# LessUp/gpu-spmv

Hardware: AMD Instinct MI355X
Metric: spmv_effective_bandwidth (higher is better)
Workload: dtype f32; 1 GPU; csr_uniform_10000000x10000000_16_per_row_pagerank_step; rows=10000000, cols=10000000, nnz=160000000, avg_nnz_per_row=16, plan_bytes=1798181216, parallelism=row-shard x1, exchange=none

## Files before the change

### gpu-spmv_amd/csrc/capi.cpp

```cpp
#include "internal.h"
#include "generators.h"
#include "pagerank_engine.h"
#include "tiled.h"
#include "spmv/bandwidth.h"
#include "spmv/bicgstab.h"
#include "spmv/gmres.h"
#include "spmv/eigs.h"
#include "spmv/cg.h"
#include "spmv/pagerank.h"
#include "spmv/sptrsv.h"
#include "spmv/ic0.h"
#include "spmv/ilu0.h"
#include "spmv/spgemm.h"
#include "spmv/amg.h"
#include "spmv/reorder.h"
#include "spmv_c.h"

#include <cstddef>
#include <cstring>
#include <vector>
#include <new>

using namespace spmv;

// ... 856 lines not shown
    sh.local_rows = A->num_rows;
    sh.map = map;
    sh.n_global = n_global;
    sh.nnz = A->nnz;
    sh.d_row_ptrs = A->d_row_ptrs;
    sh.d_cols = A->d_col_indices;
    sh.d_vals = A->d_values;
    sh.d_dangling = d_dangling_mask;
    const int partial_pairs = detail::pr_shard_prepare(&sh, detail::tiled_plan_for(A, nullptr));
    if (hipMalloc(reinterpret_cast<void**>(&sh.d_state), sizeof(detail::PrState)) != hipSuccess ||
        hipMalloc(reinterpret_cast<void**>(&sh.d_block_partials),
                  2 * sizeof(double) * static_cast<size_t>(partial_pairs)) != hipSuccess) {
        spmv_c_pr_shard_destroy(h);
        return nullptr;
    }
    return h;
}

void spmv_c_pr_shard_destroy(spmv_c_pr_shard* h) {
    if (!h) return;
    if (h->shard.commit_pending) {
        (void)detail::pr_flush(h->shard, h->shard.pending_stream);
        (void)hipGetLastError();
    }
    if (h->shard.d_state) (void)hipFree(h->shard.d_state);
    if (h->shard.d_block_partials) (void)hipFree(h->shard.d_block_partials);
    delete h;
}

int spmv_c_pr_reset(spmv_c_pr_shard* h, float dangling_sum, void* hip_stream) {
    if (!h) return kInvalidArgument;
    detail::PrState fresh{};
    fresh.dangling_sum = dangling_sum;
    h->shard.expanded_strips = 0;
    h->shard.expanded_long = false;
    detail::pr_drop_pending(h->shard);
    return hipMemcpyAsync(h->shard.d_state, &fresh, sizeof(fresh), hipMemcpyHostToDevice,
                          as_stream(hip_stream)) == hipSuccess
         ? 0 : static_cast<int>(SpMVError::CUDA_MEMCPY);
}

int spmv_c_pr_step(spmv_c_pr_shard* h, const float* d_r_old, float* d_r_new, float damping,
                   void* hip_stream) {
    if (!h || !d_r_old || !d_r_new) return kInvalidArgument;
    return launch_code(detail::pr_step(h->shard, d_r_old, d_r_new, damping, detail::PushTargets{},
                                       as_stream(hip_stream)));
}

int spmv_c_pr_step_commit(spmv_c_pr_shard* h, const float* d_r_old, float* d_r_new, float damping,
                          float tolerance, void* hip_stream) {
    if (!h || !d_r_old || !d_r_new) return kInvalidArgument;
// ... 117 lines not shown
```

### gpu-spmv_amd/csrc/pagerank.hip

```cpp
#include "internal.h"
#include "device_common.h"
#include "pagerank_engine.h"
#include "pr_commit_device.h"
#include "tiled.h"
#include "spmv/pagerank.h"

#include <hip/hip_runtime.h>

#include <algorithm>
#include <chrono>
#include <cmath>
#include <cstdio>
#include <cstdlib>
#include <cstring>
#include <mutex>
#include <vector>

namespace spmv {
namespace detail {

namespace {

using namespace dev;

// ... 122 lines not shown
__global__ __launch_bounds__(kBlock)
void pr_mask_kernel(const float* __restrict__ col_sums, int n, unsigned char* __restrict__ mask,
                    unsigned long long* __restrict__ count) {
    unsigned long long local = 0;
    for (long long c = static_cast<long long>(blockIdx.x) * kBlock + threadIdx.x; c < n;
         c += static_cast<long long>(gridDim.x) * kBlock) {
        const bool d = col_sums[c] == 0.0f;
        mask[c] = d;
        local += d;
    }
    for (int off = 32; off > 0; off >>= 1) local += __shfl_xor(local, off, 64);
    if ((threadIdx.x & 63) == 0 && local) atomicAdd(count, local);
}

__global__ __launch_bounds__(kBlock)
void pr_vector_sum_kernel(const float* __restrict__ v, size_t n, double* __restrict__ block_out) {
    double acc = 0.0, unused = 0.0;
    for (size_t i = static_cast<size_t>(blockIdx.x) * kBlock + threadIdx.x; i < n;
         i += static_cast<size_t>(gridDim.x) * kBlock) {
        acc += static_cast<double>(v[i]);
    }
    block_sum2<kBlock>(acc, unused);
    if (threadIdx.x == 0) block_out[blockIdx.x] = acc;
}

__global__ __launch_bounds__(kBlock)
void pr_scale_kernel(float* __restrict__ v, size_t n, const double* __restrict__ block_sums, int blocks) {
    __shared__ float s_total;
    if (threadIdx.x == 0) {
        double total = 0.0;
// ... 90 lines not shown
    } else if (const hipError_t e = pr_flush(sh, s); e != hipSuccess) {
        return e;
    }
    if (sh.local_rows <= 0) return hipSuccess;
    if (sh.tiled) {
        const int done = std::min(sh.expanded_strips, sh.tiled->num_strips);
        const bool long_done = sh.expanded_long;
        sh.expanded_strips = 0;
        sh.expanded_long = false;
        std::unique_lock<std::mutex> pair(sh.tiled->launch_lock, std::defer_lock);
        if (done == 0 && !long_done) pair.lock();
        if (done < sh.tiled->num_strips || !long_done) {
            const hipError_t e = tiled_pagerank_expand(*sh.tiled, done, sh.tiled->num_strips, !long_done, r_old, sh.d_state, rider, s);
            if (e != hipSuccess) return e;
        }
        return tiled_pagerank_finish(*sh.tiled, sh.map, sh.n_global, r_old, r_new, sh.d_dangling,
                                     damping, sh.d_state, sh.d_block_partials, push, s);
    }
    switch (sh.lanes) {
        case 1:  return launch_step<1>(sh, r_old, r_new, damping, push, s);
        case 2:  return launch_step<2>(sh, r_old, r_new, damping, push, s);
        case 4:  return launch_step<4>(sh, r_old, r_new, damping, push, s);
        case 8:  return launch_step<8>(sh, r_old, r_new, damping, push, s);
        case 16: return launch_step<16>(sh, r_old, r_new, damping, push, s);
        case 32: return launch_step<32>(sh, r_old, r_new, damping, push, s);
        default: return launch_step<64>(sh, r_old, r_new, damping, push, s);
    }
}

hipError_t pr_expand(const PrShard& sh, const float* r_old, long long cols_ready, hipStream_t s) {
    if (const hipError_t e = pr_flush(sh, s); e != hipSuccess) return e;
// ... 40 lines not shown
    pr_reduce_commit_kernel<<<1, kBlock, 0, s>>>(sh.d_block_partials, sh.local_rows > 0 ? sh.grid : 0, tolerance,
                                                 sh.d_state);
    return hipGetLastError();
}

hipError_t pr_commit(const PrShard& sh, const double* d_sums, float tolerance, hipStream_t s) {
    if (const hipError_t e = pr_flush(sh, s); e != hipSuccess) return e;
    pr_commit_kernel<<<1, 1, 0, s>>>(d_sums, tolerance, sh.d_state);
    return hipGetLastError();
}

hipError_t pr_commit_gathered(const PrShard& sh, const float* d_gathered, int world, long long stride,
                              long long shard_len, float tolerance, hipStream_t s) {
    if (const hipError_t e = pr_flush(sh, s); e != hipSuccess) return e;
    pr_commit_gathered_kernel<<<1, 1, 0, s>>>(d_gathered, world, stride, shard_len, tolerance, sh.d_state);
    return hipGetLastError();
}

hipError_t pr_fill(float* d_r, size_t n, float value, hipStream_t s) {
    if (n == 0) return hipSuccess;
    pr_fill_kernel<<<grid_for(static_cast<long long>(n), kBlock * 4), kBlock, 0, s>>>(d_r, n, value);
    return hipGetLastError();
}

hipError_t pr_column_sums(long long nnz, const int* d_cols, const float* d_vals, int n_cols,
                          float* d_col_sums, hipStream_t s) {
    if (nnz == 0) return hipSuccess;
    pr_colsum_kernel<<<grid_for(nnz, kBlock * 4), kBlock, 0, s>>>(nnz, d_cols, d_vals, n_cols, d_col_sums);
    return hipGetLastError();
}
// ... 463 lines not shown
```

### gpu-spmv_amd/csrc/pagerank_engine.h

```cpp
#ifndef SPMV_AMD_PAGERANK_ENGINE_H
#define SPMV_AMD_PAGERANK_ENGINE_H

#include "internal.h"

namespace spmv {
namespace detail {

struct PrState {
    float dangling_sum;
    float final_residual;
    int   iterations;
    int   converged;
    int   done;
    int   reserved;
};

constexpr int kMaxPushPeers = 15;
struct PushTargets {
    float* ptr[kMaxPushPeers];
    int count = 0;
};

struct RowMap {
    int base = 0;
    int piece = 0x7fffffff;
    int block = 0;
    __host__ __device__ long long at(long long row) const {
        return piece == 0x7fffffff ? base + row : base + (row / piece) * block + row % piece;
    }
};

struct PrShard {
    int local_rows = 0;
    RowMap map;
    int n_global = 0;
    long long nnz = 0;
    const int* d_row_ptrs = nullptr;
    const int* d_cols = nullptr;
    const float* d_vals = nullptr;
    const unsigned char* d_dangling = nullptr;
    PrState* d_state = nullptr;
    double* d_block_partials = nullptr;
    int lanes = 4;
    int grid = 1;
    PlanRef tiled;
    mutable int expanded_strips = 0;
    mutable bool expanded_long = false;
    mutable bool commit_pending = false;
    mutable float pending_tolerance = 0.0f;
    mutable hipStream_t pending_stream = nullptr;
};

struct CommitRider {
    const double* partials = nullptr;
    int num_blocks = 0;
// ... 3 lines not shown

int pr_max_blocks();
int pr_shard_prepare(PrShard* shard, PlanRef tiled);
hipError_t pr_step(const PrShard& shard, const float* d_r_old, float* d_r_new, float damping,
                   const PushTargets& push, hipStream_t s);
hipError_t pr_expand(const PrShard& shard, const float* d_r_old, long long cols_ready, hipStream_t s);
hipError_t pr_reduce(const PrShard& shard, double* d_sums , hipStream_t s);
hipError_t pr_commit(const PrShard& shard, const double* d_sums, float tolerance, hipStream_t s);
hipError_t pr_reduce_commit(const PrShard& shard, float tolerance, hipStream_t s);
hipError_t pr_step_commit(const PrShard& shard, const float* d_r_old, float* d_r_new, float damping,
                          float tolerance, hipStream_t s);
hipError_t pr_flush(const PrShard& shard, hipStream_t s);
inline void pr_drop_pending(const PrShard& shard) { shard.commit_pending = false; }
hipError_t pr_commit_gathered(const PrShard& shard, const float* d_gathered, int world, long long stride,
                              long long shard_len, float tolerance, hipStream_t s);
hipError_t pr_fill(float* d_r, size_t n, float value, hipStream_t s);
hipError_t pr_column_sums(long long nnz, const int* d_cols, const float* d_vals, int n_cols,
                          float* d_col_sums, hipStream_t s);
hipError_t pr_mask_from_column_sums(const float* d_col_sums, int n, unsigned char* d_mask,
                                    unsigned long long* d_count, hipStream_t s);

}
}

#endif
```

### gpu-spmv_amd/csrc/tiled.h

```cpp
#ifndef SPMV_AMD_TILED_H
#define SPMV_AMD_TILED_H

#include "internal.h"

#include <cstdint>
#include <mutex>
#include <vector>

namespace spmv {
namespace detail {

struct PrState;
struct CommitRider;
struct PushTargets;
struct RowMap;
struct PassDesc;

struct TiledPlan {
    int num_rows = 0, num_cols = 0;
    long long nnz = 0;
    long long entries = 0;
    int strip_cols = 0;
    int tile_rows = 0;
    int num_strips = 0, num_tiles = 0;

    DevBuf<float>    a_val;
    DevBuf<float>    col_weight;
    DevBuf<uint16_t> a_lcol;
    DevBuf<uint8_t>  a_drow;
    DevBuf<float>    prod;
    DevBuf<int>      cells_t;
    DevBuf<int>      pass_first;
    DevBuf<PassDesc> pass_desc;
    long long num_passes = 0;

    DevBuf<int> items;
    int  num_items = 0;
    std::vector<int> strip_first_item;
    DevBuf<int>   long_rows;
    int    num_long = 0;
    int    long_row = 1024;
    DevBuf<int>   long_chunks;
    int    num_long_chunks = 0;
    DevBuf<int>   long_first;
    DevBuf<float> long_sums;
    DevBuf<int>   tile_long;
    const int*   csr_row_ptrs = nullptr;
    const int*   csr_cols = nullptr;
// ... 21 lines not shown
bool tiled_eligible(const CSRMatrix* A);
bool tiled_eligible(const ELLMatrix* A);

hipError_t tiled_build(const CSRMatrix* A, TiledPlan** out, hipStream_t s);
hipError_t tiled_build(const ELLMatrix* A, TiledPlan** out, hipStream_t s);
void tiled_free(TiledPlan* plan);

hipError_t tiled_checksum(const TiledPlan& plan, unsigned long long out[4], hipStream_t s);

hipError_t tiled_spmv(const TiledPlan& plan, const float* d_x, float* d_y, hipStream_t s);

hipError_t tiled_pagerank_expand(const TiledPlan& plan, int strip_begin, int strip_end, bool with_long,
                                 const float* d_r_old, const PrState* d_state, const CommitRider& commit, hipStream_t s);
hipError_t tiled_pagerank_finish(const TiledPlan& plan, const RowMap& map, int n_global,
                                 const float* d_r_old, float* d_r_new,
                                 const unsigned char* d_dangling, float damping,
                                 const PrState* d_state, double* d_block_partials,
                                 const PushTargets& push, hipStream_t s);

}
}

#endif
```

### gpu-spmv_amd/csrc/tiled.hip

```cpp
#include "tiled.h"
#include "tiled_layout.h"
#include "device_common.h"
#include "pagerank_engine.h"
#include "pr_commit_device.h"

#include <hip/hip_runtime.h>

#include <algorithm>
#include <mutex>

namespace spmv {
namespace detail {

namespace {

using namespace dev;

typedef unsigned short u16x4 __attribute__((ext_vector_type(4)));

template <typename T>
__device__ __forceinline__ void store_product(T* p, T v) { __builtin_nontemporal_store(v, p); }

struct LongRows {
    const int* chunks;
// ... 74 lines not shown
                *reinterpret_cast<f32x4*>(xs + i) = *reinterpret_cast<const f32x4*>(src + i);
            } else {
                for (int k = i; k < width; ++k) xs[k] = src[k];
            }
        }
    } else {
        for (int i = threadIdx.x; i < width; i += kExpandBlock) xs[i] = src[i];
    }
}

template <int kExpandBlock, bool FOLD>
__device__ __forceinline__ void expand_slots(const float* xs, int begin, int end, const float* __restrict__ a_val,
                                             const unsigned short* __restrict__ a_lcol, float* __restrict__ prod) {
    constexpr int kStride = kExpandBlock * 4;
    if (FOLD) {
        for (int q = (begin & ~3) + threadIdx.x * 4; q < end; q += 2 * kStride) {
#pragma unroll
            for (int u = 0; u < 2; ++u) {
                const int g = q + u * kStride;
                if (g >= begin && g + 3 < end) {
                    const u16x4 c = *reinterpret_cast<const u16x4*>(a_lcol + g);
                    f32x4 p;
                    p[0] = xs[c[0]]; p[1] = xs[c[1]]; p[2] = xs[c[2]]; p[3] = xs[c[3]];
                    store_product(reinterpret_cast<f32x4*>(prod + g), p);
                } else {
                    for (int k = max(g, begin); k < min(g + 4, end); ++k) prod[k] = xs[a_lcol[k]];
                }
            }
        }
        return;
    }
    for (int q = (begin & ~3) + threadIdx.x * 4; q < end; q += kStride) {
        if (q >= begin && q + 3 < end) {
            const u16x4 c = *reinterpret_cast<const u16x4*>(a_lcol + q);
            const f32x4 v = *reinterpret_cast<const f32x4*>(a_val + q);
            f32x4 p;
            p[0] = v[0] * xs[c[0]];
            p[1] = v[1] * xs[c[1]];
            p[2] = v[2] * xs[c[2]];
            p[3] = v[3] * xs[c[3]];
            store_product(reinterpret_cast<f32x4*>(prod + q), p);
        } else {
            for (int k = max(q, begin); k < min(q + 4, end); ++k) prod[k] = a_val[k] * xs[a_lcol[k]];
        }
    }
}

// ... 27 lines not shown
    stage_strip<W, kExpandBlock, FOLD>(xs, x, col_weight, static_cast<long long>(strip) * W, num_cols);
    __syncthreads();
    expand_slots<kExpandBlock, FOLD>(xs, begin, end, a_val, a_lcol, prod);
}

struct LongSeeds {
    const int* rows;
    const int* first_chunk;
    const int* tile_first;
    const float* chunk_sum;
};

__device__ __forceinline__ void tile_accumulate(double* tile, int R, int tile_index,
                                                const int* __restrict__ pass_first, const PassDesc* __restrict__ desc,
                                                const float* __restrict__ prod,
                                                const unsigned char* __restrict__ a_drow,
                                                const LongSeeds seeds) {
    __shared__ double spare[64];
    const long long first = static_cast<long long>(tile_index) * R;
    for (int i = threadIdx.x; i < R; i += kReduceThreads) tile[i] = 0.0;
    if (seeds.tile_first) {
        __syncthreads();
        for (int k = seeds.tile_first[tile_index] + threadIdx.x; k < seeds.tile_first[tile_index + 1]; k += kReduceThreads) {
            double total = 0.0;
            for (int c = seeds.first_chunk[k]; c < seeds.first_chunk[k + 1]; ++c) total += static_cast<double>(seeds.chunk_sum[c]);
            tile[seeds.rows[k] - first] = total;
        }
    }
    __syncthreads();

    const int wave = __builtin_amdgcn_readfirstlane(static_cast<int>(threadIdx.x >> 6));
    const int lane = threadIdx.x & 63;
    const int pass_lo = pass_first[tile_index * kReduceWaves + wave], pass_hi = pass_first[tile_index * kReduceWaves + wave + 1];

    struct Pass {
        int lane_adj;
        int groups;
        f32x4 p;
        unsigned int d;
    };
    for (int window_first = pass_lo; window_first < pass_hi; window_first += 64) {
        const uint4* mine = reinterpret_cast<const uint4*>(desc + window_first + min(lane, pass_hi - window_first - 1));
        uint4 lo = mine[0], hi = mine[1];
        asm volatile("; pass descriptors settled" : "+v"(lo.x), "+v"(lo.y), "+v"(lo.z), "+v"(lo.w), "+v"(hi.x), "+v"(hi.y), "+v"(hi.z));
        const int window_passes = min(64, pass_hi - window_first);

        auto open = [&](Pass& ps, int k) {
            const int idx = __builtin_amdgcn_readfirstlane(k);
            const int base0 = __builtin_amdgcn_readlane(static_cast<int>(lo.x), idx);
            const int base1 = __builtin_amdgcn_readlane(static_cast<int>(lo.y), idx);
            const int base2 = __builtin_amdgcn_readlane(static_cast<int>(lo.z), idx);
            const int adj0 = __builtin_amdgcn_readlane(static_cast<int>(lo.w), idx);
            const int adj1 = __builtin_amdgcn_readlane(static_cast<int>(hi.x), idx);
            const int adj2 = __builtin_amdgcn_readlane(static_cast<int>(hi.y), idx);
            const unsigned int geom = static_cast<unsigned int>(__builtin_amdgcn_readlane(static_cast<int>(hi.z), idx));
            const int start1 = static_cast<int>(geom & 0xFF), start2 = static_cast<int>((geom >> 8) & 0xFF);
            ps.groups = static_cast<int>(geom >> 16);
            const int at = min(lane, ps.groups - 1);
            int base = base0, adj = adj0;
            base = at >= start1 ? base1 : base;
            adj = at >= start1 ? adj1 : adj;
            base = at >= start2 ? base2 : base;
            adj = at >= start2 ? adj2 : adj;
            ps.lane_adj = adj;
            const unsigned int slot = static_cast<unsigned int>(base + 4 * at);
            ps.p = *reinterpret_cast<const f32x4*>(reinterpret_cast<const char*>(prod) + (static_cast<size_t>(slot) << 2));
            ps.d = *reinterpret_cast<const unsigned int*>(a_drow + slot);
        };
        auto add = [&](const Pass& ps) {
            const unsigned int word = lane < ps.groups ? ps.d : 0xFFFFFFFFu;
            int delta[4], upto[4], sum = 0;
#pragma unroll
            for (int e = 0; e < 4; ++e) {
                delta[e] = (word >> (8 * e)) & 0xFF;
                sum += delta[e];
                upto[e] = sum;
            }
            const int incl = wave_inclusive_scan(sum);
            const int lane_base = ps.lane_adj + incl - sum;
#pragma unroll
            for (int e = 0; e < 4; ++e) {
                double* target = delta[e] != kSkip ? &tile[lane_base + upto[e]] : &spare[lane];
                atomicAdd(target, static_cast<double>(ps.p[e]));
            }
        };
// ... 21 lines not shown
                if (k + u + kPassDepth < window_passes) open(ps[u], k + u + kPassDepth);
            }
        }
#pragma unroll
        for (int u = 0; u < kPassDepth; ++u) {
            if (k + kPassDepth + u < window_passes) add(ps[u]);
        }
    }
    __syncthreads();
}

template <int kReduceBlock>
__global__ __launch_bounds__(kReduceBlock, kReduceBlock / 128)
void tiled_reduce_kernel(int R, int num_tiles, const int* __restrict__ pass_first, const PassDesc* __restrict__ pass_desc,
                         const float* __restrict__ prod,
                         const unsigned char* __restrict__ a_drow,
                         const LongSeeds seeds,
                         int num_rows, float* __restrict__ y) {
    static_assert(kReduceBlock == kReduceThreads, "the pass layout is made for this workgroup size");
    extern __shared__ double tile[];
    const int tile_index = xcd_contiguous(blockIdx.x, num_tiles);
    if (tile_index < 0) return;
    tile_accumulate(tile, R, tile_index, pass_first, pass_desc, prod, a_drow, seeds);
    const long long first = static_cast<long long>(tile_index) * R;
    for (int i = threadIdx.x; i < R && first + i < num_rows; i += kReduceBlock) y[first + i] = static_cast<float>(tile[i]);
}

template <int kReduceBlock>
__global__ __launch_bounds__(kReduceBlock, kReduceBlock / 128)
void tiled_pagerank_reduce_kernel(int R, int num_tiles, const int* __restrict__ pass_first, const PassDesc* __restrict__ pass_desc,
                                  const float* __restrict__ prod,
                                  const unsigned char* __restrict__ a_drow,
                                  const LongSeeds seeds,
                                  int local_rows, RowMap map, int n_global,
                                  const float* __restrict__ r_old, float* __restrict__ r_new,
                                  const unsigned char* __restrict__ dangling, float damping,
                                  const PrState* __restrict__ state,
                                  double* __restrict__ block_partials, PushTargets push) {
    if (state->done) return;
    extern __shared__ double tile[];
    const int tile_index = xcd_contiguous(blockIdx.x, num_tiles);
    if (tile_index < 0) return;
    tile_accumulate(tile, R, tile_index, pass_first, pass_desc, prod, a_drow, seeds);

    const float teleport = __fdiv_rn(1.0f - damping, static_cast<float>(n_global));
    const float dangling_term = __fdiv_rn(__fmul_rn(damping, state->dangling_sum),
                                          static_cast<float>(n_global));
    double res2 = 0.0, mass = 0.0;
    const long long first = static_cast<long long>(tile_index) * R;
    if (map.piece == 0x7fffffff && push.count == 0) {
        constexpr int kPerThread = (kMaxTileRows + kReduceBlock - 1) / kReduceBlock;
        const long long node_first = map.base + first;
        const int rows_here = static_cast<int>(min(static_cast<long long>(R), local_rows - first));
        float old_rank[kPerThread];
        unsigned char is_dangling[kPerThread];
#pragma unroll
        for (int u = 0; u < kPerThread; ++u) {
            const int i = min(static_cast<int>(threadIdx.x) + u * kReduceBlock, rows_here - 1);
            old_rank[u] = r_old[node_first + i];
            is_dangling[u] = dangling[node_first + i];
        }
#pragma unroll
        for (int u = 0; u < kPerThread; ++u) {
            const int i = threadIdx.x + u * kReduceBlock;
            if (i < rows_here) {
                const float fresh = __fadd_rn(__fadd_rn(__fmul_rn(damping, static_cast<float>(tile[i])), dangling_term), teleport);
                r_new[node_first + i] = fresh;
                const float diff = __fsub_rn(fresh, old_rank[u]);
                res2 += static_cast<double>(__fmul_rn(diff, diff));
                if (is_dangling[u]) mass += static_cast<double>(fresh);
            }
        }
    } else {
        for (int i = threadIdx.x; i < R && first + i < local_rows; i += kReduceBlock) {
            const long long node = map.at(first + i);
            const float fresh = __fadd_rn(__fadd_rn(__fmul_rn(damping, static_cast<float>(tile[i])), dangling_term), teleport);
            r_new[node] = fresh;
            for (int p = 0; p < push.count; ++p) push.ptr[p][node] = fresh;
            const float diff = __fsub_rn(fresh, r_old[node]);
            res2 += static_cast<double>(__fmul_rn(diff, diff));
            if (dangling[node]) mass += static_cast<double>(fresh);
        }
    }
    block_sum2<kReduceBlock>(res2, mass);
    if (threadIdx.x == 0) {
// ... 70 lines not shown
        constexpr int BLOCK = W <= 16384 ? 512 : 1024;
        return launch_expand_as<W, BLOCK>(plan, sc, first_item, num_items, with_long, d_x, d_state, commit, s);
    });
}

LongSeeds long_seeds(const TiledPlan& plan, const Scratch& sc) {
    return LongSeeds{plan.long_rows.get(), plan.long_first.get(), plan.num_long > 0 ? plan.tile_long.get() : nullptr, sc.long_sums};
}

hipError_t launch_reduce(const TiledPlan& plan, const Scratch& sc, float* d_y, hipStream_t s) {
    const size_t lds = static_cast<size_t>(plan.tile_rows) * sizeof(double);
    const void* kernel = reinterpret_cast<const void*>(&tiled_reduce_kernel<kReduceThreads>);
    const hipError_t e = hipFuncSetAttribute(kernel, hipFuncAttributeMaxDynamicSharedMemorySize, static_cast<int>(lds));
    if (e != hipSuccess) return e;
    tiled_reduce_kernel<kReduceThreads><<<xcd_grid(plan.num_tiles), kReduceThreads, lds, s>>>(
        plan.tile_rows, plan.num_tiles, plan.pass_first.get(), plan.pass_desc.get(), sc.prod, plan.a_drow.get(),
        long_seeds(plan, sc), plan.num_rows, d_y);
    return hipGetLastError();
}

hipError_t launch_pagerank_reduce(const TiledPlan& plan, const Scratch& sc, const RowMap& map, int n_global, const float* d_r_old,
                                  float* d_r_new, const unsigned char* d_dangling, float damping,
                                  const PrState* d_state, double* d_block_partials,
                                  const PushTargets& push, hipStream_t s) {
    const size_t lds = static_cast<size_t>(plan.tile_rows) * sizeof(double);
    const void* kernel = reinterpret_cast<const void*>(&tiled_pagerank_reduce_kernel<kReduceThreads>);
    const hipError_t e = hipFuncSetAttribute(kernel, hipFuncAttributeMaxDynamicSharedMemorySize, static_cast<int>(lds));
    if (e != hipSuccess) return e;
    tiled_pagerank_reduce_kernel<kReduceThreads><<<xcd_grid(plan.num_tiles), kReduceThreads, lds, s>>>(
        plan.tile_rows, plan.num_tiles, plan.pass_first.get(), plan.pass_desc.get(), sc.prod, plan.a_drow.get(),
        long_seeds(plan, sc), plan.num_rows, map, n_global, d_r_old, d_r_new, d_dangling, damping, d_state,
        d_block_partials, push);
    return hipGetLastError();
}

}

hipError_t tiled_spmv(const TiledPlan& plan, const float* d_x, float* d_y, hipStream_t s) {
    Scratch sc;
    hipError_t e = scratch_for(plan, s, &sc);
    if (e != hipSuccess) return e;
    std::lock_guard<std::mutex> pair(plan.launch_lock);
    e = launch_expand(plan, sc, 0, plan.num_items, true, d_x, nullptr, CommitRider{}, s);
    if (e != hipSuccess) return e;
    return launch_reduce(plan, sc, d_y, s);
}

hipError_t tiled_pagerank_expand(const TiledPlan& plan, int strip_begin, int strip_end, bool with_long,
                                 const float* d_r_old, const PrState* d_state, const CommitRider& commit, hipStream_t s) {
    Scratch sc;
    const hipError_t e = scratch_for(plan, s, &sc);
    if (e != hipSuccess) return e;
    strip_begin = std::max(0, std::min(strip_begin, plan.num_strips));
    strip_end = std::max(strip_begin, std::min(strip_end, plan.num_strips));
    const int first = plan.strip_first_item[strip_begin];
    return launch_expand(plan, sc, first, plan.strip_first_item[strip_end] - first, with_long, d_r_old, d_state, commit, s);
}

hipError_t tiled_pagerank_finish(const TiledPlan& plan, const RowMap& map, int n_global,
                                 const float* d_r_old, float* d_r_new,
                                 const unsigned char* d_dangling, float damping,
                                 const PrState* d_state, double* d_block_partials,
                                 const PushTargets& push, hipStream_t s) {
    Scratch sc;
    const hipError_t e = scratch_for(plan, s, &sc);
    if (e != hipSuccess) return e;
    return launch_pagerank_reduce(plan, sc, map, n_global, d_r_old, d_r_new, d_dangling, damping, d_state,
                                  d_block_partials, push, s);
}

}
}
```

### gpu-spmv_amd/csrc/tiled_build.hip

```cpp
#include "tiled_build.h"
#include "tiled_layout.h"
#include "device_common.h"

#include <hip/hip_runtime.h>

#include <algorithm>
#include <chrono>
#include <cstdlib>
#include <memory>
#include <vector>

namespace spmv {
namespace detail {

namespace {

using namespace dev;

constexpr int kMaxItemEntries = 16384;
constexpr int kMinItemEntries = 4096;
constexpr int kMaxLongRow = 4096;

constexpr unsigned int kNoWeight = 0x7FC0BEEFu;
template <int W>
// ... 39 lines not shown
        }
    }
    if (PASS == 1 && bad) *differs = 1;
}

__global__ __launch_bounds__(kBlock)
void weight_finish_kernel(float* __restrict__ weight, int n) {
    for (long long i = static_cast<long long>(blockIdx.x) * kBlock + threadIdx.x; i < n;
         i += static_cast<long long>(gridDim.x) * kBlock) {
        if (__float_as_uint(weight[i]) == kNoWeight) weight[i] = 0.0f;
    }
}

__global__ __launch_bounds__(kBlock)
void plan_checksum_kernel(long long slots, const float* __restrict__ a_val, const unsigned short* __restrict__ a_lcol,
                          const unsigned char* __restrict__ a_drow, long long table_ints, const int* __restrict__ cells_t,
                          unsigned long long* __restrict__ out ) {
    unsigned long long v = 0, c = 0, d = 0, t = 0;
    for (long long i = static_cast<long long>(blockIdx.x) * kBlock + threadIdx.x; i < slots;
         i += static_cast<long long>(gridDim.x) * kBlock) {
        const unsigned long long w = 2 * static_cast<unsigned long long>(i) + 1;
        if (a_val) v += w * __float_as_uint(a_val[i]);
        c += w * a_lcol[i];
        d += w * a_drow[i];
    }
    for (long long i = static_cast<long long>(blockIdx.x) * kBlock + threadIdx.x; i < table_ints;
         i += static_cast<long long>(gridDim.x) * kBlock) {
        t += (2 * static_cast<unsigned long long>(i) + 1) * static_cast<unsigned int>(cells_t[i]);
    }
    for (int off = 32; off > 0; off >>= 1) {
        v += __shfl_xor(v, off, 64);
        c += __shfl_xor(c, off, 64);
        d += __shfl_xor(d, off, 64);
        t += __shfl_xor(t, off, 64);
    }
    if ((threadIdx.x & 63) == 0) {
        atomicAdd(&out[0], v);
        atomicAdd(&out[1], c);
        atomicAdd(&out[2], d);
// ... 164 lines not shown
    plan->long_row = A ? std::max(64, std::min(long_cap, long_factor * plan->num_strips)) : 0x3fffffff;

    bool fold = true;
    if (const char* env = std::getenv("SPMV_TILED_FOLD")) fold = env[0] != '0';
    BuiltCells built;
    hipError_t e = A ? build_cells(A, plan.get(), &built, s) : build_cells(src.ell, plan.get(), &built, s);
    trace.mark("cells built, temporaries freed");
    if (e == hipSuccess) e = layout_passes(plan.get(), s);
    if (e != hipSuccess) return e;
    trace.mark("phase-2 pass descriptors");

    if (A && plan->num_long > 0) e = cut_long_rows(A, plan.get());
    if (e == hipSuccess && fold && plan->nnz > 0) e = probe_fold(plan.get(), built.strip_begin.get(), s);
    if (e != hipSuccess) return e;
    built.strip_begin.reset();

    e = dev_alloc(&plan->prod, plan->nnz + 8);
    if (e == hipSuccess) e = make_items(plan.get(), built.host_strip);
    if (e != hipSuccess) return e;

    trace.mark("fold probe, long rows, items");
    plan->plan_bytes = plan->nnz * (4  + 2 + 1 + (plan->a_val ? 4 : 0)) + cells * 8 +
                       plan->num_passes * static_cast<long long>(sizeof(PassDesc)) + 4LL * (plan->num_tiles * kReduceWaves + 1) +
                       (plan->col_weight ? 4LL * plan->num_cols : 0) +
                       12LL * plan->num_items + 12LL * plan->num_long_chunks;
    plan->build_ms = std::chrono::duration<double, std::milli>(std::chrono::steady_clock::now() - t_begin).count();
    *out = plan.release();
    return hipSuccess;
}

}

hipError_t tiled_build(const CSRMatrix* A, TiledPlan** out, hipStream_t s) {
    Source src;
    src.csr = A;
    src.rows = A->num_rows;
    src.cols = A->num_cols;
    src.nnz = A->nnz;
// ... 6 lines not shown
    src.rows = A->num_rows;
    src.cols = A->num_cols;
    src.nnz = static_cast<long long>(A->num_rows) * A->max_nnz_per_row;
    return build_plan(src, out, s);
}


void tiled_free(TiledPlan* p) { delete p; }

hipError_t tiled_checksum(const TiledPlan& plan, unsigned long long out[4], hipStream_t s) {
    DevBuf<unsigned long long> d_out;
    hipError_t e = dev_alloc(&d_out, 4);
    if (e != hipSuccess) return e;
    e = hipMemsetAsync(d_out.get(), 0, 4 * sizeof(unsigned long long), s);
    if (e == hipSuccess) {
        plan_checksum_kernel<<<1024, kBlock, 0, s>>>(plan.nnz, plan.a_val.get(), plan.a_lcol.get(), plan.a_drow.get(),
                                                     2LL * plan.num_strips * plan.num_tiles, plan.cells_t.get(), d_out.get());
        e = hipGetLastError();
    }
    if (e == hipSuccess) e = hipMemcpyAsync(out, d_out.get(), 4 * sizeof(unsigned long long), hipMemcpyDeviceToHost, s);
    if (e == hipSuccess) e = hipStreamSynchronize(s);
    return e;
}

}
}
```

### gpu-spmv_amd/csrc/tiled_cells.hip

```cpp
#include "tiled_build.h"
#include "tiled_layout.h"
#include "device_common.h"

#include <hip/hip_runtime.h>

#include <algorithm>

namespace spmv {
namespace detail {

namespace {

using namespace dev;

constexpr int kBuildBlock = 1024;
constexpr int kBuildRowCache = 1024;
constexpr int kBuildLdsSmall = 70 * 1024;
constexpr int kBuildLdsLarge = 148 * 1024;
constexpr int kBuildBinWords = 4;
constexpr int kBuildEntryBytes = 11;
constexpr int kBuildWaveCountBytes = kBuildBlock / 64;

struct CsrSource {
    const int* row_ptrs;
// ... 811 lines not shown
    for (long long i = static_cast<long long>(blockIdx.x) * kBlock + threadIdx.x; i <= cells;
         i += static_cast<long long>(gridDim.x) * kBlock) {
        if (i < cells) {
            const long long tile = i / num_strips, strip = i % num_strips;
            const long long cell = strip * num_tiles + tile;
            cells_t[i] = make_int2(offs[cell], offs[cell + 1] - offs[cell]);
        }
        if (i <= num_strips) strip_begin[i] = offs[i * num_tiles];
    }
}

template <bool FILL>
__global__ __launch_bounds__(kReduceThreads)
void pass_layout_kernel(int num_tiles, int num_strips, const int2* __restrict__ cells_t,
                        const unsigned char* __restrict__ a_drow,
                        int* __restrict__ pass_count, const int* __restrict__ pass_first, PassDesc* __restrict__ desc) {
    const int tile_index = blockIdx.x;
    if (tile_index >= num_tiles) return;
    const int wave = __builtin_amdgcn_readfirstlane(static_cast<int>(threadIdx.x >> 6));
    const int lane = threadIdx.x & 63;
    int run_lo, run_hi;
    wave_runs(num_strips, wave, &run_lo, &run_hi);
    const int2* mine = cells_t + static_cast<long long>(tile_index) * num_strips;
    int passes = 0;
    long long out = FILL ? pass_first[tile_index * kReduceWaves + wave] : 0;
    for (int window_first = run_lo; window_first < run_hi; window_first += 64) {
        const int2 window = window_first + lane < run_hi ? mine[window_first + lane] : make_int2(0, 0);
        const int window_runs = min(64, run_hi - window_first);
        int next_run = 0, cur_begin = 0, cur_len = 0, off = 0;
        int row_carry = 0;
        for (;;) {
// ... 14 lines not shown
                start[k] = filled >> 2;
                last = take > 0 ? k : last;
                filled += take;
                off += take;
            }
            if (filled == 0) break;
            ++passes;
            if (!FILL) continue;
            const bool open_end = off < cur_len;
            const int groups = filled >> 2;
            const int at = min(lane, groups - 1);
            int mine_base = base[0];
#pragma unroll
            for (int k = 1; k < kPassSegs; ++k) mine_base = at >= start[k] ? base[k] : mine_base;
            const unsigned int word = lane < groups ? *reinterpret_cast<const unsigned int*>(a_drow + mine_base + 4 * at) : 0u;
            const int sum = static_cast<int>((word & 0xFF) + ((word >> 8) & 0xFF) + ((word >> 16) & 0xFF) + (word >> 24));
            const int incl = wave_inclusive_scan(sum);
            int adj[kPassSegs];
            int origin = fresh0 ? 0 : row_carry;
            adj[0] = origin;
#pragma unroll
            for (int k = 1; k < kPassSegs; ++k) {
                const int before = start[k] > 0 ? __builtin_amdgcn_readlane(incl, max(start[k] - 1, 0)) : 0;
                adj[k] = -before;
                origin = k <= last ? adj[k] : origin;
            }
            row_carry = open_end ? origin + __builtin_amdgcn_readlane(incl, groups - 1) : 0;
            if (lane == 0) {
                PassDesc d;
#pragma unroll
// ... 139 lines not shown
    e = dev_alloc(&plan->a_val, plan->nnz + 8);
    if (e == hipSuccess) e = dev_alloc(&plan->a_lcol, plan->nnz + 8);
    if (e == hipSuccess) e = dev_alloc(&plan->a_drow, plan->nnz + 8);
    if (e == hipSuccess) e = dev_alloc(&plan->cells_t, 2 * cells);
    const int pass_waves = T * kReduceWaves;
    if (e == hipSuccess) e = dev_alloc(&plan->pass_first, static_cast<long long>(pass_waves) + 1);
    if (e != hipSuccess) return e;
    float* a_val = plan->a_val.get();
    unsigned short* a_lcol = plan->a_lcol.get();
    unsigned char* a_drow = plan->a_drow.get();
    int2* cells_t = reinterpret_cast<int2*>(plan->cells_t.get());
    int* pass_first = plan->pass_first.get();
    {
        const int grid = static_cast<int>(std::min<long long>((cells + kBlock) / kBlock, 4096));
        cell_table_kernel<<<grid, kBlock, 0, s>>>(offs, S, T, cells_t, strip_begin);
        pass_layout_kernel<false><<<T, kReduceThreads, 0, s>>>(T, S, cells_t, nullptr, pass_first, nullptr, nullptr);
        exclusive_scan_small_kernel<<<1, kScanBlock, 0, s>>>(pass_first, pass_waves);
    }
    if (plan->nnz > 0) {
        bool staged = true;
        if (debug_is("place", "scattered")) staged = false;
        int* todo = place_todo;
        if (staged) {
            const int stage_slots = (capacity + 1024 + 63) / 64 * 64;
            const size_t stage_lds = static_cast<size_t>(kStageBytesPerStrip) * S + static_cast<size_t>(kStageBytesPerSlot) * stage_slots;
            staged = stage_lds + sizeof(int) * kBuildBlock + 64 <= 160 * 1024;
            if (staged) e = hipMemsetAsync(todo, 0, sizeof(int), s);
            if (staged && e == hipSuccess) {
                e = hipFuncSetAttribute(reinterpret_cast<const void*>(&batch_place_staged_kernel<Src>),
                                        hipFuncAttributeMaxDynamicSharedMemorySize, static_cast<int>(stage_lds));
            }
// ... 22 lines not shown
}

}

hipError_t build_cells(const CSRMatrix* A, TiledPlan* plan, BuiltCells* out, hipStream_t s) {
    const CsrSource dev_src{A->d_row_ptrs, A->d_col_indices, A->d_values};
    return build_cells_from(dev_src, true, plan, out, s);
}

hipError_t build_cells(const ELLMatrix* A, TiledPlan* plan, BuiltCells* out, hipStream_t s) {
    const EllSource dev_src{A->num_rows, A->max_nnz_per_row, A->d_col_indices, A->d_values};
    return build_cells_from(dev_src, false, plan, out, s);
}

hipError_t layout_passes(TiledPlan* plan, hipStream_t s) {
    const hipError_t e = dev_alloc(&plan->pass_desc, plan->num_passes);
    if (e != hipSuccess) return e;
    pass_layout_kernel<true><<<plan->num_tiles, kReduceThreads, 0, s>>>(plan->num_tiles, plan->num_strips,
                                                                       reinterpret_cast<const int2*>(plan->cells_t.get()), plan->a_drow.get(), nullptr,
                                                                       plan->pass_first.get(), plan->pass_desc.get());
    return hipGetLastError();
}

}
}
```

### gpu-spmv_amd/csrc/tiled_layout.h

```cpp
#ifndef SPMV_AMD_TILED_LAYOUT_H
#define SPMV_AMD_TILED_LAYOUT_H

#include <type_traits>

namespace spmv {
namespace detail {

template <class F>
auto with_strip_width(int strip_cols, F&& f) {
    switch (strip_cols) {
        case 4096:  return f(std::integral_constant<int, 4096>{});
        case 8192:  return f(std::integral_constant<int, 8192>{});
        case 16384: return f(std::integral_constant<int, 16384>{});
        default:    return f(std::integral_constant<int, 32768>{});
    }
}

constexpr int kSkip = 255;
constexpr int kLongChunk = 512;
constexpr long long kMaxCells = 1LL << 26;
constexpr long long kResidentTiles = 512;
constexpr int kMaxTileRows = 9984;
constexpr int kMaxBuildStrips = 3072;

constexpr int kPassSegs = 3;
constexpr int kPassSlots = 256;
constexpr int kPassDepth = 3;
constexpr int kReduceThreads = 1024;
constexpr int kReduceWaves = kReduceThreads / 64;

struct PassDesc {
    int base[kPassSegs];
    int adj[kPassSegs];
    unsigned int geom;
    unsigned int reserved;
};
static_assert(sizeof(PassDesc) == 32, "a lane loads its pass descriptor as two 16-byte words");

#ifdef __HIP__
constexpr int kXcds = 8;
__device__ __forceinline__ int xcd_contiguous(int block, int count) {
    const int per_xcd = (count + kXcds - 1) / kXcds;
    const int which = (block % kXcds) * per_xcd + block / kXcds;
    return block / kXcds < per_xcd && which < count ? which : -1;
}
__host__ __device__ inline int xcd_grid(int count) { return (count + kXcds - 1) / kXcds * kXcds; }

__device__ __forceinline__ void wave_runs(int num_strips, int wave, int* lo, int* hi) {
    const int per_wave = (num_strips + kReduceWaves - 1) / kReduceWaves;
    *lo = min(num_strips, wave * per_wave);
    *hi = min(num_strips, *lo + per_wave);
}
#endif
// ... 6 lines not shown
```

Measured before the change: 2921 GB/s.

## Pack per-pass row-delta words and bit-pack dangling flags for PageRank reduce

```diff
diff --git a/gpu-spmv_amd/csrc/capi.cpp b/gpu-spmv_amd/csrc/capi.cpp
--- a/gpu-spmv_amd/csrc/capi.cpp
+++ b/gpu-spmv_amd/csrc/capi.cpp
@@ -894,6 +894,17 @@
         spmv_c_pr_shard_destroy(h);
         return nullptr;
     }
+    if (sh.tiled && sh.local_rows > 0 && piece == 0x7fffffff && !detail::debug_is("dangling", "bytes")) {
+        hipStream_t s = detail::current_stream();
+        if (hipMalloc(reinterpret_cast<void**>(&sh.d_dangling_words),
+                      sizeof(unsigned int) * detail::pr_dangling_words(sh.local_rows)) != hipSuccess ||
+            hipMalloc(reinterpret_cast<void**>(&sh.d_tile_dangling), sizeof(int) * static_cast<size_t>(sh.tiled->num_tiles)) != hipSuccess ||
+            detail::pr_dangling_bits(&sh, s) != hipSuccess || hipStreamSynchronize(s) != hipSuccess) {
+            (void)hipGetLastError();
+            spmv_c_pr_shard_destroy(h);
+            return nullptr;
+        }
+    }
     return h;
 }
 
@@ -905,6 +916,8 @@
     }
     if (h->shard.d_state) (void)hipFree(h->shard.d_state);
     if (h->shard.d_block_partials) (void)hipFree(h->shard.d_block_partials);
+    if (h->shard.d_dangling_words) (void)hipFree(h->shard.d_dangling_words);
+    if (h->shard.d_tile_dangling) (void)hipFree(h->shard.d_tile_dangling);
     delete h;
 }
 
@@ -915,6 +928,7 @@
     h->shard.expanded_strips = 0;
     h->shard.expanded_long = false;
     detail::pr_drop_pending(h->shard);
+    if (detail::pr_dangling_bits(&h->shard, as_stream(hip_stream)) != hipSuccess) return kLaunch;
     return hipMemcpyAsync(h->shard.d_state, &fresh, sizeof(fresh), hipMemcpyHostToDevice,
                           as_stream(hip_stream)) == hipSuccess
          ? 0 : static_cast<int>(SpMVError::CUDA_MEMCPY);
diff --git a/gpu-spmv_amd/csrc/pagerank.hip b/gpu-spmv_amd/csrc/pagerank.hip
--- a/gpu-spmv_amd/csrc/pagerank.hip
+++ b/gpu-spmv_amd/csrc/pagerank.hip
@@ -160,6 +160,22 @@
 }
 
 __global__ __launch_bounds__(kBlock)
+void pr_dangling_bits_kernel(const unsigned char* __restrict__ mask, int rows, int R,
+                             unsigned int* __restrict__ words, int* __restrict__ tile_count) {
+    const long long padded = (static_cast<long long>(rows) + 63) / 64 * 64;
+    for (long long i = static_cast<long long>(blockIdx.x) * kBlock + threadIdx.x; i < padded;
+         i += static_cast<long long>(gridDim.x) * kBlock) {
+        const bool flag = i < rows && mask[i] != 0;
+        const unsigned long long set = __ballot(flag);
+        if ((threadIdx.x & 63) == 0) {
+            words[i >> 5] = static_cast<unsigned int>(set);
+            words[(i >> 5) + 1] = static_cast<unsigned int>(set >> 32);
+            if (set) atomicAdd(&tile_count[i / R], __popcll(set));
+        }
+    }
+}
+
+__global__ __launch_bounds__(kBlock)
 void pr_vector_sum_kernel(const float* __restrict__ v, size_t n, double* __restrict__ block_out) {
     double acc = 0.0, unused = 0.0;
     for (size_t i = static_cast<size_t>(blockIdx.x) * kBlock + threadIdx.x; i < n;
@@ -280,7 +296,8 @@
             const hipError_t e = tiled_pagerank_expand(*sh.tiled, done, sh.tiled->num_strips, !long_done, r_old, sh.d_state, rider, s);
             if (e != hipSuccess) return e;
         }
-        return tiled_pagerank_finish(*sh.tiled, sh.map, sh.n_global, r_old, r_new, sh.d_dangling,
+        const DanglingBits bits = sh.dangling_bits_ready ? DanglingBits{sh.d_dangling_words, sh.d_tile_dangling} : DanglingBits{};
+        return tiled_pagerank_finish(*sh.tiled, sh.map, sh.n_global, r_old, r_new, sh.d_dangling, bits,
                                      damping, sh.d_state, sh.d_block_partials, push, s);
     }
     switch (sh.lanes) {
@@ -351,6 +368,18 @@
                               long long shard_len, float tolerance, hipStream_t s) {
     if (const hipError_t e = pr_flush(sh, s); e != hipSuccess) return e;
     pr_commit_gathered_kernel<<<1, 1, 0, s>>>(d_gathered, world, stride, shard_len, tolerance, sh.d_state);
+    return hipGetLastError();
+}
+
+hipError_t pr_dangling_bits(PrShard* sh, hipStream_t s) {
+    sh->dangling_bits_ready = false;
+    if (!sh->d_dangling_words || !sh->d_tile_dangling || !sh->tiled || sh->map.piece != 0x7fffffff || sh->local_rows <= 0) return hipSuccess;
+    const TiledPlan& plan = *sh->tiled;
+    const hipError_t e = hipMemsetAsync(sh->d_tile_dangling, 0, sizeof(int) * static_cast<size_t>(plan.num_tiles), s);
+    if (e != hipSuccess) return e;
+    pr_dangling_bits_kernel<<<grid_for(sh->local_rows, kBlock * 4), kBlock, 0, s>>>(
+        sh->d_dangling + sh->map.base, sh->local_rows, plan.tile_rows, sh->d_dangling_words, sh->d_tile_dangling);
+    sh->dangling_bits_ready = true;
     return hipGetLastError();
 }
 
diff --git a/gpu-spmv_amd/csrc/pagerank_engine.h b/gpu-spmv_amd/csrc/pagerank_engine.h
--- a/gpu-spmv_amd/csrc/pagerank_engine.h
+++ b/gpu-spmv_amd/csrc/pagerank_engine.h
@@ -2,6 +2,8 @@
 #define SPMV_AMD_PAGERANK_ENGINE_H
 
 #include "internal.h"
+
+#include <algorithm>
 
 namespace spmv {
 namespace detail {
@@ -30,6 +32,12 @@
     }
 };
 
+struct DanglingBits {
+    const unsigned int* words = nullptr;
+    const int* tile_count = nullptr;
+};
+inline size_t pr_dangling_words(int local_rows) { return 2 * ((static_cast<size_t>(std::max(local_rows, 0)) + 63) / 64); }
+
 struct PrShard {
     int local_rows = 0;
     RowMap map;
@@ -39,6 +47,9 @@
     const int* d_cols = nullptr;
     const float* d_vals = nullptr;
     const unsigned char* d_dangling = nullptr;
+    unsigned int* d_dangling_words = nullptr;
+    int* d_tile_dangling = nullptr;
+    bool dangling_bits_ready = false;
     PrState* d_state = nullptr;
     double* d_block_partials = nullptr;
     int lanes = 4;
@@ -72,6 +83,7 @@
 inline void pr_drop_pending(const PrShard& shard) { shard.commit_pending = false; }
 hipError_t pr_commit_gathered(const PrShard& shard, const float* d_gathered, int world, long long stride,
                               long long shard_len, float tolerance, hipStream_t s);
+hipError_t pr_dangling_bits(PrShard* shard, hipStream_t s);
 hipError_t pr_fill(float* d_r, size_t n, float value, hipStream_t s);
 hipError_t pr_column_sums(long long nnz, const int* d_cols, const float* d_vals, int n_cols,
                           float* d_col_sums, hipStream_t s);
diff --git a/gpu-spmv_amd/csrc/tiled.h b/gpu-spmv_amd/csrc/tiled.h
--- a/gpu-spmv_amd/csrc/tiled.h
+++ b/gpu-spmv_amd/csrc/tiled.h
@@ -14,6 +14,7 @@
 struct CommitRider;
 struct PushTargets;
 struct RowMap;
+struct DanglingBits;
 struct PassDesc;
 
 struct TiledPlan {
@@ -32,6 +33,7 @@
     DevBuf<int>      cells_t;
     DevBuf<int>      pass_first;
     DevBuf<PassDesc> pass_desc;
+    DevBuf<uint32_t> pass_word;
     long long num_passes = 0;
 
     DevBuf<int> items;
@@ -83,7 +85,7 @@
                                  const float* d_r_old, const PrState* d_state, const CommitRider& commit, hipStream_t s);
 hipError_t tiled_pagerank_finish(const TiledPlan& plan, const RowMap& map, int n_global,
                                  const float* d_r_old, float* d_r_new,
-                                 const unsigned char* d_dangling, float damping,
+                                 const unsigned char* d_dangling, const DanglingBits& bits, float damping,
                                  const PrState* d_state, double* d_block_partials,
                                  const PushTargets& push, hipStream_t s);
 
diff --git a/gpu-spmv_amd/csrc/tiled.hip b/gpu-spmv_amd/csrc/tiled.hip
--- a/gpu-spmv_amd/csrc/tiled.hip
+++ b/gpu-spmv_amd/csrc/tiled.hip
@@ -112,7 +112,7 @@
                                              const unsigned short* __restrict__ a_lcol, float* __restrict__ prod) {
     constexpr int kStride = kExpandBlock * 4;
     if (FOLD) {
-        for (int q = (begin & ~3) + threadIdx.x * 4; q < end; q += 2 * kStride) {
+        for (int q = (begin & ~15) + threadIdx.x * 4; q < end; q += 2 * kStride) {
 #pragma unroll
             for (int u = 0; u < 2; ++u) {
                 const int g = q + u * kStride;
@@ -128,7 +128,7 @@
         }
         return;
     }
-    for (int q = (begin & ~3) + threadIdx.x * 4; q < end; q += kStride) {
+    for (int q = (begin & ~15) + threadIdx.x * 4; q < end; q += kStride) {
         if (q >= begin && q + 3 < end) {
             const u16x4 c = *reinterpret_cast<const u16x4*>(a_lcol + q);
             const f32x4 v = *reinterpret_cast<const f32x4*>(a_val + q);
@@ -186,7 +186,7 @@
 __device__ __forceinline__ void tile_accumulate(double* tile, int R, int tile_index,
                                                 const int* __restrict__ pass_first, const PassDesc* __restrict__ desc,
                                                 const float* __restrict__ prod,
-                                                const unsigned char* __restrict__ a_drow,
+                                                const unsigned int* __restrict__ pass_word,
                                                 const LongSeeds seeds) {
     __shared__ double spare[64];
     const long long first = static_cast<long long>(tile_index) * R;
@@ -207,7 +207,6 @@
 
     struct Pass {
         int lane_adj;
-        int groups;
         f32x4 p;
         unsigned int d;
     };
@@ -227,8 +226,9 @@
             const int adj2 = __builtin_amdgcn_readlane(static_cast<int>(hi.y), idx);
             const unsigned int geom = static_cast<unsigned int>(__builtin_amdgcn_readlane(static_cast<int>(hi.z), idx));
             const int start1 = static_cast<int>(geom & 0xFF), start2 = static_cast<int>((geom >> 8) & 0xFF);
-            ps.groups = static_cast<int>(geom >> 16);
-            const int at = min(lane, ps.groups - 1);
+            const int groups = static_cast<int>(geom >> 16);
+            ps.d = pass_word[(static_cast<size_t>(window_first) + idx) * 64 + lane];
+            const int at = min(lane, groups - 1);
             int base = base0, adj = adj0;
             base = at >= start1 ? base1 : base;
             adj = at >= start1 ? adj1 : adj;
@@ -237,10 +237,9 @@
             ps.lane_adj = adj;
             const unsigned int slot = static_cast<unsigned int>(base + 4 * at);
             ps.p = *reinterpret_cast<const f32x4*>(reinterpret_cast<const char*>(prod) + (static_cast<size_t>(slot) << 2));
-            ps.d = *reinterpret_cast<const unsigned int*>(a_drow + slot);
         };
         auto add = [&](const Pass& ps) {
-            const unsigned int word = lane < ps.groups ? ps.d : 0xFFFFFFFFu;
+            const unsigned int word = ps.d;
             int delta[4], upto[4], sum = 0;
 #pragma unroll
             for (int e = 0; e < 4; ++e) {
@@ -292,14 +291,14 @@
 __global__ __launch_bounds__(kReduceBlock, kReduceBlock / 128)
 void tiled_reduce_kernel(int R, int num_tiles, const int* __restrict__ pass_first, const PassDesc* __restrict__ pass_desc,
                          const float* __restrict__ prod,
-                         const unsigned char* __restrict__ a_drow,
+                         const unsigned int* __restrict__ pass_word,
                          const LongSeeds seeds,
                          int num_rows, float* __restrict__ y) {
     static_assert(kReduceBlock == kReduceThreads, "the pass layout is made for this workgroup size");
     extern __shared__ double tile[];
     const int tile_index = xcd_contiguous(blockIdx.x, num_tiles);
     if (tile_index < 0) return;
-    tile_accumulate(tile, R, tile_index, pass_first, pass_desc, prod, a_drow, seeds);
+    tile_accumulate(tile, R, tile_index, pass_first, pass_desc, prod, pass_word, seeds);
     const long long first = static_cast<long long>(tile_index) * R;
     for (int i = threadIdx.x; i < R && first + i < num_rows; i += kReduceBlock) y[first + i] = static_cast<float>(tile[i]);
 }
@@ -308,18 +307,19 @@
 __global__ __launch_bounds__(kReduceBlock, kReduceBlock / 128)
 void tiled_pagerank_reduce_kernel(int R, int num_tiles, const int* __restrict__ pass_first, const PassDesc* __restrict__ pass_desc,
                                   const float* __restrict__ prod,
-                                  const unsigned char* __restrict__ a_drow,
+                                  const unsigned int* __restrict__ pass_word,
                                   const LongSeeds seeds,
                                   int local_rows, RowMap map, int n_global,
                                   const float* __restrict__ r_old, float* __restrict__ r_new,
-                                  const unsigned char* __restrict__ dangling, float damping,
+                                  const unsigned char* __restrict__ dangling, DanglingBits bits, float damping,
                                   const PrState* __restrict__ state,
                                   double* __restrict__ block_partials, PushTargets push) {
     if (state->done) return;
     extern __shared__ double tile[];
     const int tile_index = xcd_contiguous(blockIdx.x, num_tiles);
     if (tile_index < 0) return;
-    tile_accumulate(tile, R, tile_index, pass_first, pass_desc, prod, a_drow, seeds);
+    const int flagged_rows = bits.words ? bits.tile_count[tile_index] : 0;
+    tile_accumulate(tile, R, tile_index, pass_first, pass_desc, prod, pass_word, seeds);
 
     const float teleport = __fdiv_rn(1.0f - damping, static_cast<float>(n_global));
     const float dangling_term = __fdiv_rn(__fmul_rn(damping, state->dangling_sum),
@@ -331,12 +331,29 @@
         const long long node_first = map.base + first;
         const int rows_here = static_cast<int>(min(static_cast<long long>(R), local_rows - first));
         float old_rank[kPerThread];
-        unsigned char is_dangling[kPerThread];
+        unsigned int is_dangling[kPerThread];
 #pragma unroll
         for (int u = 0; u < kPerThread; ++u) {
             const int i = min(static_cast<int>(threadIdx.x) + u * kReduceBlock, rows_here - 1);
             old_rank[u] = r_old[node_first + i];
-            is_dangling[u] = dangling[node_first + i];
+        }
+        const bool packed = bits.words != nullptr;
+        const unsigned int flag_shift = packed ? threadIdx.x & 31u : 0u;
+        if (!packed) {
+#pragma unroll
+            for (int u = 0; u < kPerThread; ++u) {
+                const int i = min(static_cast<int>(threadIdx.x) + u * kReduceBlock, rows_here - 1);
+                is_dangling[u] = dangling[node_first + i];
+            }
+        } else if (flagged_rows != 0) {
+#pragma unroll
+            for (int u = 0; u < kPerThread; ++u) {
+                const long long row = first + min(static_cast<int>(threadIdx.x) + u * kReduceBlock, rows_here - 1);
+                is_dangling[u] = bits.words[row >> 5];
+            }
+        } else {
+#pragma unroll
+            for (int u = 0; u < kPerThread; ++u) is_dangling[u] = 0;
         }
 #pragma unroll
         for (int u = 0; u < kPerThread; ++u) {
@@ -346,7 +363,7 @@
                 r_new[node_first + i] = fresh;
                 const float diff = __fsub_rn(fresh, old_rank[u]);
                 res2 += static_cast<double>(__fmul_rn(diff, diff));
-                if (is_dangling[u]) mass += static_cast<double>(fresh);
+                if (packed ? (is_dangling[u] >> flag_shift) & 1u : is_dangling[u]) mass += static_cast<double>(fresh);
             }
         }
     } else {
@@ -447,13 +464,13 @@
     const hipError_t e = hipFuncSetAttribute(kernel, hipFuncAttributeMaxDynamicSharedMemorySize, static_cast<int>(lds));
     if (e != hipSuccess) return e;
     tiled_reduce_kernel<kReduceThreads><<<xcd_grid(plan.num_tiles), kReduceThreads, lds, s>>>(
-        plan.tile_rows, plan.num_tiles, plan.pass_first.get(), plan.pass_desc.get(), sc.prod, plan.a_drow.get(),
+        plan.tile_rows, plan.num_tiles, plan.pass_first.get(), plan.pass_desc.get(), sc.prod, plan.pass_word.get(),
         long_seeds(plan, sc), plan.num_rows, d_y);
     return hipGetLastError();
 }
 
 hipError_t launch_pagerank_reduce(const TiledPlan& plan, const Scratch& sc, const RowMap& map, int n_global, const float* d_r_old,
-                                  float* d_r_new, const unsigned char* d_dangling, float damping,
+                                  float* d_r_new, const unsigned char* d_dangling, const DanglingBits& bits, float damping,
                                   const PrState* d_state, double* d_block_partials,
                                   const PushTargets& push, hipStream_t s) {
     const size_t lds = static_cast<size_t>(plan.tile_rows) * sizeof(double);
@@ -461,8 +478,8 @@
     const hipError_t e = hipFuncSetAttribute(kernel, hipFuncAttributeMaxDynamicSharedMemorySize, static_cast<int>(lds));
     if (e != hipSuccess) return e;
     tiled_pagerank_reduce_kernel<kReduceThreads><<<xcd_grid(plan.num_tiles), kReduceThreads, lds, s>>>(
-        plan.tile_rows, plan.num_tiles, plan.pass_first.get(), plan.pass_desc.get(), sc.prod, plan.a_drow.get(),
-        long_seeds(plan, sc), plan.num_rows, map, n_global, d_r_old, d_r_new, d_dangling, damping, d_state,
+        plan.tile_rows, plan.num_tiles, plan.pass_first.get(), plan.pass_desc.get(), sc.prod, plan.pass_word.get(),
+        long_seeds(plan, sc), plan.num_rows, map, n_global, d_r_old, d_r_new, d_dangling, bits, damping, d_state,
         d_block_partials, push);
     return hipGetLastError();
 }
@@ -492,13 +509,13 @@
 
 hipError_t tiled_pagerank_finish(const TiledPlan& plan, const RowMap& map, int n_global,
                                  const float* d_r_old, float* d_r_new,
-                                 const unsigned char* d_dangling, float damping,
+                                 const unsigned char* d_dangling, const DanglingBits& bits, float damping,
                                  const PrState* d_state, double* d_block_partials,
                                  const PushTargets& push, hipStream_t s) {
     Scratch sc;
     const hipError_t e = scratch_for(plan, s, &sc);
     if (e != hipSuccess) return e;
-    return launch_pagerank_reduce(plan, sc, map, n_global, d_r_old, d_r_new, d_dangling, damping, d_state,
+    return launch_pagerank_reduce(plan, sc, map, n_global, d_r_old, d_r_new, d_dangling, bits, damping, d_state,
                                   d_block_partials, push, s);
 }
 
diff --git a/gpu-spmv_amd/csrc/tiled_build.hip b/gpu-spmv_amd/csrc/tiled_build.hip
--- a/gpu-spmv_amd/csrc/tiled_build.hip
+++ b/gpu-spmv_amd/csrc/tiled_build.hip
@@ -77,7 +77,8 @@
 
 __global__ __launch_bounds__(kBlock)
 void plan_checksum_kernel(long long slots, const float* __restrict__ a_val, const unsigned short* __restrict__ a_lcol,
-                          const unsigned char* __restrict__ a_drow, long long table_ints, const int* __restrict__ cells_t,
+                          long long delta_words, const unsigned int* __restrict__ pass_word,
+                          long long table_ints, const int* __restrict__ cells_t,
                           unsigned long long* __restrict__ out ) {
     unsigned long long v = 0, c = 0, d = 0, t = 0;
     for (long long i = static_cast<long long>(blockIdx.x) * kBlock + threadIdx.x; i < slots;
@@ -85,7 +86,10 @@
         const unsigned long long w = 2 * static_cast<unsigned long long>(i) + 1;
         if (a_val) v += w * __float_as_uint(a_val[i]);
         c += w * a_lcol[i];
-        d += w * a_drow[i];
+    }
+    for (long long i = static_cast<long long>(blockIdx.x) * kBlock + threadIdx.x; i < delta_words;
+         i += static_cast<long long>(gridDim.x) * kBlock) {
+        d += (2 * static_cast<unsigned long long>(i) + 1) * pass_word[i];
     }
     for (long long i = static_cast<long long>(blockIdx.x) * kBlock + threadIdx.x; i < table_ints;
          i += static_cast<long long>(gridDim.x) * kBlock) {
@@ -280,14 +284,16 @@
     if (e == hipSuccess && fold && plan->nnz > 0) e = probe_fold(plan.get(), built.strip_begin.get(), s);
     if (e != hipSuccess) return e;
     built.strip_begin.reset();
+    plan->a_drow.reset();
 
     e = dev_alloc(&plan->prod, plan->nnz + 8);
     if (e == hipSuccess) e = make_items(plan.get(), built.host_strip);
     if (e != hipSuccess) return e;
 
     trace.mark("fold probe, long rows, items");
-    plan->plan_bytes = plan->nnz * (4  + 2 + 1 + (plan->a_val ? 4 : 0)) + cells * 8 +
-                       plan->num_passes * static_cast<long long>(sizeof(PassDesc)) + 4LL * (plan->num_tiles * kReduceWaves + 1) +
+    plan->plan_bytes = plan->nnz * (4  + 2 + (plan->a_val ? 4 : 0)) + cells * 8 +
+                       plan->num_passes * static_cast<long long>(sizeof(PassDesc) + kPassSlots ) +
+                       4LL * (plan->num_tiles * kReduceWaves + 1) +
                        (plan->col_weight ? 4LL * plan->num_cols : 0) +
                        12LL * plan->num_items + 12LL * plan->num_long_chunks;
     plan->build_ms = std::chrono::duration<double, std::milli>(std::chrono::steady_clock::now() - t_begin).count();
@@ -324,8 +330,9 @@
     if (e != hipSuccess) return e;
     e = hipMemsetAsync(d_out.get(), 0, 4 * sizeof(unsigned long long), s);
     if (e == hipSuccess) {
-        plan_checksum_kernel<<<1024, kBlock, 0, s>>>(plan.nnz, plan.a_val.get(), plan.a_lcol.get(), plan.a_drow.get(),
-                                                     2LL * plan.num_strips * plan.num_tiles, plan.cells_t.get(), d_out.get());
+        plan_checksum_kernel<<<1024, kBlock, 0, s>>>(plan.nnz, plan.a_val.get(), plan.a_lcol.get(), 64 * plan.num_passes,
+                                                     plan.pass_word.get(), 2LL * plan.num_strips * plan.num_tiles,
+                                                     plan.cells_t.get(), d_out.get());
         e = hipGetLastError();
     }
     if (e == hipSuccess) e = hipMemcpyAsync(out, d_out.get(), 4 * sizeof(unsigned long long), hipMemcpyDeviceToHost, s);
diff --git a/gpu-spmv_amd/csrc/tiled_cells.hip b/gpu-spmv_amd/csrc/tiled_cells.hip
--- a/gpu-spmv_amd/csrc/tiled_cells.hip
+++ b/gpu-spmv_amd/csrc/tiled_cells.hip
@@ -849,7 +849,8 @@
 __global__ __launch_bounds__(kReduceThreads)
 void pass_layout_kernel(int num_tiles, int num_strips, const int2* __restrict__ cells_t,
                         const unsigned char* __restrict__ a_drow,
-                        int* __restrict__ pass_count, const int* __restrict__ pass_first, PassDesc* __restrict__ desc) {
+                        int* __restrict__ pass_count, const int* __restrict__ pass_first, PassDesc* __restrict__ desc,
+                        unsigned int* __restrict__ pass_word) {
     const int tile_index = blockIdx.x;
     if (tile_index >= num_tiles) return;
     const int wave = __builtin_amdgcn_readfirstlane(static_cast<int>(threadIdx.x >> 6));
@@ -894,6 +895,7 @@
 #pragma unroll
             for (int k = 1; k < kPassSegs; ++k) mine_base = at >= start[k] ? base[k] : mine_base;
             const unsigned int word = lane < groups ? *reinterpret_cast<const unsigned int*>(a_drow + mine_base + 4 * at) : 0u;
+            pass_word[out * 64 + lane] = lane < groups ? word : 0xFFFFFFFFu;
             const int sum = static_cast<int>((word & 0xFF) + ((word >> 8) & 0xFF) + ((word >> 16) & 0xFF) + (word >> 24));
             const int incl = wave_inclusive_scan(sum);
             int adj[kPassSegs];
@@ -1063,7 +1065,7 @@
     {
         const int grid = static_cast<int>(std::min<long long>((cells + kBlock) / kBlock, 4096));
         cell_table_kernel<<<grid, kBlock, 0, s>>>(offs, S, T, cells_t, strip_begin);
-        pass_layout_kernel<false><<<T, kReduceThreads, 0, s>>>(T, S, cells_t, nullptr, pass_first, nullptr, nullptr);
+        pass_layout_kernel<false><<<T, kReduceThreads, 0, s>>>(T, S, cells_t, nullptr, pass_first, nullptr, nullptr, nullptr);
         exclusive_scan_small_kernel<<<1, kScanBlock, 0, s>>>(pass_first, pass_waves);
     }
     if (plan->nnz > 0) {
@@ -1116,11 +1118,12 @@
 }
 
 hipError_t layout_passes(TiledPlan* plan, hipStream_t s) {
-    const hipError_t e = dev_alloc(&plan->pass_desc, plan->num_passes);
+    hipError_t e = dev_alloc(&plan->pass_desc, plan->num_passes);
+    if (e == hipSuccess) e = dev_alloc(&plan->pass_word, 64 * plan->num_passes);
     if (e != hipSuccess) return e;
     pass_layout_kernel<true><<<plan->num_tiles, kReduceThreads, 0, s>>>(plan->num_tiles, plan->num_strips,
                                                                        reinterpret_cast<const int2*>(plan->cells_t.get()), plan->a_drow.get(), nullptr,
-                                                                       plan->pass_first.get(), plan->pass_desc.get());
+                                                                       plan->pass_first.get(), plan->pass_desc.get(), plan->pass_word.get());
     return hipGetLastError();
 }
 
diff --git a/gpu-spmv_amd/csrc/tiled_layout.h b/gpu-spmv_amd/csrc/tiled_layout.h
--- a/gpu-spmv_amd/csrc/tiled_layout.h
+++ b/gpu-spmv_amd/csrc/tiled_layout.h
@@ -37,6 +37,7 @@
 };
 static_assert(sizeof(PassDesc) == 32, "a lane loads its pass descriptor as two 16-byte words");
 
+
 #ifdef __HIP__
 constexpr int kXcds = 8;
 __device__ __forceinline__ int xcd_contiguous(int block, int count) {
```

Measured after the change: 2964 GB/s, median of 6. +1.5%, better.
